# AvalonEnjoyer/pytorch-ViT-paper-replication

Hardware: AMD Instinct MI355X
Metric: images/sec (whole node) ViT-B/16 224px bf16 at 1/2/4/8 MI355X (higher is better)
Workload: dtype bf16; 1 GPU; model=ViT-B/16, global_batch=256, per_gpu_batch=256, seq_len=197, image_size=224, parallelism=dp1, impl=fused, grad_transport=none, optimizer=Adam(wd=0.03 decay group) + clip 1.0 + warmup/linear-decay LR, dropout=0.1 (mlp, embedding)

## Files before the change

### pytorch_vit_paper_replication_amd/csrc/layernorm.hip

```cpp
#include "common.h"
#include "kernels.h"

namespace pvr {
namespace {

template <int MAXCH>
__global__ void __launch_bounds__(256) ln_fwd_kernel(const uint16_t* __restrict__ x, int64_t x_stride,
                                                      const float* __restrict__ w, const float* __restrict__ b,
                                                      uint16_t* __restrict__ y, int64_t y_stride,
                                                      float* __restrict__ mean_out, float* __restrict__ rstd_out,
                                                      int rows, int D, float eps) {
  const int lane = threadIdx.x & 63;
  const int row = blockIdx.x * 4 + (threadIdx.x >> 6);
  if (row >= rows) return;
  const int nch = D >> 3;
  PVR_ASSERT((D & 7) == 0 && nch <= 64 * MAXCH);
  const uint16_t* xr = x + (int64_t)row * x_stride;
  float v[MAXCH][8];
  float s = 0.f;
#pragma unroll
  for (int i = 0; i < MAXCH; ++i) {
    const int c = lane + 64 * i;
    if (c < nch) {
      const uint4 q = *(const uint4*)(xr + c * 8);
      const uint32_t u[4] = {q.x, q.y, q.z, q.w};
#pragma unroll
      for (int j = 0; j < 4; ++j) {
        v[i][2 * j] = bf2f(u[j] & 0xFFFF);
        v[i][2 * j + 1] = bf2f(u[j] >> 16);
      }
#pragma unroll
      for (int j = 0; j < 8; ++j) s += v[i][j];
    } else {
#pragma unroll
      for (int j = 0; j < 8; ++j) v[i][j] = 0.f;
    }
  }
  const float mean = wave_sum(s) / D;
  float ss = 0.f;
#pragma unroll
  for (int i = 0; i < MAXCH; ++i) {
    const int c = lane + 64 * i;
    if (c < nch) {
#pragma unroll
      for (int j = 0; j < 8; ++j) {
        const float d = v[i][j] - mean;
        ss += d * d;
      }
    }
  }
  const float rstd = rsqrtf(wave_sum(ss) / D + eps);
  uint16_t* yr = y + (int64_t)row * y_stride;
#pragma unroll
  for (int i = 0; i < MAXCH; ++i) {
    const int c = lane + 64 * i;
    if (c < nch) {
      const float4 w0 = *(const float4*)(w + c * 8), w1 = *(const float4*)(w + c * 8 + 4);
      const float4 b0 = *(const float4*)(b + c * 8), b1 = *(const float4*)(b + c * 8 + 4);
      const float ww[8] = {w0.x, w0.y, w0.z, w0.w, w1.x, w1.y, w1.z, w1.w};
      const float bb[8] = {b0.x, b0.y, b0.z, b0.w, b1.x, b1.y, b1.z, b1.w};
      float o[8];
#pragma unroll
      for (int j = 0; j < 8; ++j) o[j] = (v[i][j] - mean) * rstd * ww[j] + bb[j];
      uint4 q;
      q.x = pack2bf(o[0], o[1]); q.y = pack2bf(o[2], o[3]);
      q.z = pack2bf(o[4], o[5]); q.w = pack2bf(o[6], o[7]);
      *(uint4*)(yr + c * 8) = q;
    }
  }
  if (lane == 0) {
    mean_out[row] = mean;
    rstd_out[row] = rstd;
  }
}

template <int MAXCH>
__global__ void __launch_bounds__(256) ln_fwd_q8_kernel(const uint16_t* __restrict__ x, int64_t x_stride,
                                                        const float* __restrict__ w, const float* __restrict__ b,
                                                        uint16_t* __restrict__ y, int64_t y_stride, uint8_t* __restrict__ yq,
                                                        int64_t q_stride, const float* __restrict__ qscale,
                                                        unsigned* __restrict__ amax, float* __restrict__ mean_out,
                                                        float* __restrict__ rstd_out, int rows, int D, float eps) {
  __shared__ float wm[4];
  const int lane = threadIdx.x & 63;
  const int nch = D >> 3;
  const float qs = *qscale;
  float am = 0.f;
  for (int row = blockIdx.x * 4 + (int)(threadIdx.x >> 6); row < rows; row += gridDim.x * 4) {
    const uint16_t* xr = x + (int64_t)row * x_stride;
    float v[MAXCH][8];
    float s = 0.f;
#pragma unroll
    for (int i = 0; i < MAXCH; ++i) {
      const int c = lane + 64 * i;
      if (c < nch) {
        const uint4 q = *(const uint4*)(xr + c * 8);
        const uint32_t u[4] = {q.x, q.y, q.z, q.w};
#pragma unroll
        for (int j = 0; j < 4; ++j) {
          v[i][2 * j] = bf2f(u[j] & 0xFFFF);
          v[i][2 * j + 1] = bf2f(u[j] >> 16);
        }
#pragma unroll
        for (int j = 0; j < 8; ++j) s += v[i][j];
      } else {
#pragma unroll
        for (int j = 0; j < 8; ++j) v[i][j] = 0.f;
      }
    }
    const float mean = wave_sum(s) / D;
    float ss = 0.f;
#pragma unroll
    for (int i = 0; i < MAXCH; ++i) {
      const int c = lane + 64 * i;
      if (c < nch) {
#pragma unroll
        for (int j = 0; j < 8; ++j) {
          const float d = v[i][j] - mean;
          ss += d * d;
        }
      }
    }
    const float rstd = rsqrtf(wave_sum(ss) / D + eps);
    uint16_t* yr = y ? y + (int64_t)row * y_stride : nullptr;
    uint8_t* qr = yq + (int64_t)row * q_stride;
#pragma unroll
    for (int i = 0; i < MAXCH; ++i) {
      const int c = lane + 64 * i;
      if (c < nch) {
        const float4 w0 = *(const float4*)(w + c * 8), w1 = *(const float4*)(w + c * 8 + 4);
        const float4 b0 = *(const float4*)(b + c * 8), b1 = *(const float4*)(b + c * 8 + 4);
        const float ww[8] = {w0.x, w0.y, w0.z, w0.w, w1.x, w1.y, w1.z, w1.w};
        const float bb[8] = {b0.x, b0.y, b0.z, b0.w, b1.x, b1.y, b1.z, b1.w};
        float o[8];
        float vm = 0.f;
#pragma unroll
        for (int j = 0; j < 8; ++j) {
          o[j] = (v[i][j] - mean) * rstd * ww[j] + bb[j];
          vm = nan_max(vm, fabsf(o[j]));
        }
        am = nan_max(am, vm);
        uint4 q;
        q.x = pack2bf(o[0], o[1]); q.y = pack2bf(o[2], o[3]);
        q.z = pack2bf(o[4], o[5]); q.w = pack2bf(o[6], o[7]);
        if (yr) *(uint4*)(yr + c * 8) = q;
        *(uint2*)(qr + c * 8) = pack8_fp8_fast<0>(o, qs, vm);
      }
    }
    if (lane == 0) {
      mean_out[row] = mean;
      rstd_out[row] = rstd;
    }
  }
  am = wave_max_nan(am);
  if (lane == 0) wm[threadIdx.x >> 6] = am;
  __syncthreads();
  if (threadIdx.x == 0) {
    const float m = nan_max(nan_max(wm[0], wm[1]), nan_max(wm[2], wm[3]));
    if (!(m <= 0.f)) atomicMax(amax, __float_as_uint(m));
  }
}

PVR_DEV void load8(const uint16_t* p, float* o) {
  const uint4 q = *(const uint4*)p;
  const uint32_t u[4] = {q.x, q.y, q.z, q.w};
#pragma unroll
  for (int j = 0; j < 4; ++j) {
    o[2 * j] = bf2f(u[j] & 0xFFFF);
    o[2 * j + 1] = bf2f(u[j] >> 16);
  }
}

template <int W>
struct RowVec;
template <>
struct RowVec<8> {
  uint32_t u[4];
  PVR_DEV void load(const uint16_t* p) { const uint4 q = *(const uint4*)p; u[0] = q.x; u[1] = q.y; u[2] = q.z; u[3] = q.w; }
  PVR_DEV void store(uint16_t* p) const { *(uint4*)p = make_uint4(u[0], u[1], u[2], u[3]); }
  PVR_DEV void zero() { u[0] = u[1] = u[2] = u[3] = 0u; }
};
template <>
struct RowVec<4> {
  uint32_t u[2];
  PVR_DEV void load(const uint16_t* p) { const uint2 q = *(const uint2*)p; u[0] = q.x; u[1] = q.y; }
  PVR_DEV void store(uint16_t* p) const { *(uint2*)p = make_uint2(u[0], u[1]); }
  PVR_DEV void zero() { u[0] = u[1] = 0u; }
};

template <int MAXCH, int W, bool Q8, bool SP, bool DP = false>
__global__ void __launch_bounds__(256) ln_bwd_kernel(const uint16_t* __restrict__ dy, int64_t dy_stride,
                                                      const uint16_t* __restrict__ x, int64_t x_stride,
                                                      const float* __restrict__ mean, const float* __restrict__ rstd,
                                                      const float* __restrict__ w,
                                                      const uint16_t* __restrict__ dres, int64_t dres_stride,
                                                      uint16_t* __restrict__ dx, int64_t dx_stride,
                                                      float* __restrict__ dw, float* __restrict__ db, float* __restrict__ dsum,
                                                      float* __restrict__ part,
                                                      uint16_t* __restrict__ dz, int64_t dz_stride,
                                                      const uint64_t* __restrict__ seed_ptr, uint64_t seed_off, uint32_t thr,
                                                      float dscale, int dz_nostore, uint8_t* __restrict__ qout, int64_t q_stride,
                                                      const float* __restrict__ qscale, unsigned* __restrict__ amax, int qfmt,
                                                      int rows, int D, int dres_every,
                                                      const uint64_t* __restrict__ dp_seed_ptr, uint64_t dp_off, uint32_t dp_thr,
                                                      float dp_scale, int dp_rows) {
  __shared__ float red[4][MAXCH * 64 * W > 1280 ? 1280 : MAXCH * 64 * W];
  __shared__ float qred[4];
  const float qs = Q8 ? *qscale : 1.f;
  float qam = 0.f;
  const int lane = threadIdx.x & 63, wave = threadIdx.x >> 6;
  const int nch = D / W;
  float gw[MAXCH][W], gb[MAXCH][W], gs[MAXCH][W];
#pragma unroll
  for (int i = 0; i < MAXCH; ++i)
#pragma unroll
    for (int j = 0; j < W; ++j) gw[i][j] = gb[i][j] = gs[i][j] = 0.f;

  const int stride = gridDim.x * 4;
  RowVec<W> cx[MAXCH], cdy[MAXCH], cr[MAXCH];
  auto load_row = [&](int row, RowVec<W> (&qx)[MAXCH], RowVec<W> (&qd)[MAXCH], RowVec<W> (&qr)[MAXCH]) {
    const int rr = min(row, rows - 1);
#pragma unroll
    for (int i = 0; i < MAXCH; ++i) {
      const int c = min(lane + 64 * i, nch - 1);
      qx[i].load(x + (int64_t)rr * x_stride + c * W);
      qd[i].load(dy + (int64_t)rr * dy_stride + c * W);
      if constexpr (SP) {
        qr[i].load(dres + (int64_t)(rr / dres_every) * dres_stride + c * W);
        if (rr % dres_every) qr[i].zero();
      } else if (dres)
        qr[i].load(dres + (int64_t)rr * dres_stride + c * W);
      else
        qr[i].zero();
    }
  };
  float wreg[MAXCH][W];
#pragma unroll
  for (int i = 0; i < MAXCH; ++i) {
    const int c = min(lane + 64 * i, nch - 1);
#pragma unroll
    for (int j = 0; j < W; j += 4) {
      const float4 w4 = *(const float4*)(w + c * W + j);
      wreg[i][j] = w4.x; wreg[i][j + 1] = w4.y; wreg[i][j + 2] = w4.z; wreg[i][j + 3] = w4.w;
    }
  }
  const uint64_t seed = dz && (!DP || thr) ? *seed_ptr + seed_off : 0ull;
  uint32_t dkey = 0u;
  float dfk = 0.f;
  if constexpr (DP) {
    dkey = rng_key(*dp_seed_ptr + dp_off);
    dfk = (thr ? dscale : 1.f) * dp_scale;
  }
  int row = blockIdx.x * 4 + wave;
  load_row(row, cx, cdy, cr);
  float cmu = row < rows ? mean[row] : 0.f, crs = row < rows ? rstd[row] : 0.f;
  for (; row < rows; row += stride) {
    RowVec<W> nx[MAXCH], ndy[MAXCH], nr[MAXCH];
    load_row(row + stride, nx, ndy, nr);
    const int rn = min(row + stride, rows - 1);
    const float nmu = mean[rn], nrs = rstd[rn];
    const float mu = cmu, rs = crs;
    auto xhat = [&](int i, int j) { return (bf2f(j & 1 ? cx[i].u[j >> 1] >> 16 : cx[i].u[j >> 1] & 0xFFFF) - mu) * rs; };
    auto dyv = [&](int i, int j) { return bf2f(j & 1 ? cdy[i].u[j >> 1] >> 16 : cdy[i].u[j >> 1] & 0xFFFF); };
    float s1 = 0.f, s2 = 0.f;
#pragma unroll
    for (int i = 0; i < MAXCH; ++i) {
      const int c = lane + 64 * i;
      if (c < nch) {
#pragma unroll
        for (int j = 0; j < W; ++j) {
          const float xh = xhat(i, j), dv = dyv(i, j);
          const float g = dv * wreg[i][j];
          s1 += g;
          s2 += g * xh;
          gw[i][j] += dv * xh;
          gb[i][j] += dv;
        }
      }
    }
    const float c1 = wave_sum(s1) / D, c2 = wave_sum(s2) / D;
#pragma unroll
    for (int i = 0; i < MAXCH; ++i) {
      const int c = lane + 64 * i;
      if (c < nch) {
        float o[W];
#pragma unroll
        for (int j = 0; j < W; ++j) o[j] = (dyv(i, j) * wreg[i][j] - c1 - xhat(i, j) * c2) * rs;
        if (dres) {
#pragma unroll
          for (int j = 0; j < W; ++j) o[j] += bf2f(j & 1 ? cr[i].u[j >> 1] >> 16 : cr[i].u[j >> 1] & 0xFFFF);
        }
        RowVec<W> q;
#pragma unroll
        for (int j = 0; j < W; j += 2) q.u[j >> 1] = pack2bf(o[j], o[j + 1]);
        q.store(dx + (int64_t)row * dx_stride + c * W);
        if (dz) {
          if constexpr (DP) {
            const float rf = rng_keep_32(dkey, (uint32_t)row / (uint32_t)dp_rows, dp_thr) ? dfk : 0.f;
#pragma unroll
            for (int j = 0; j < W; j += 2) {
              bool k0 = true, k1 = true;
              if (thr) rng_keep2(seed, (uint64_t)row * D + c * W + j, thr, k0, k1);
              o[j] = k0 ? o[j] * rf : 0.f;
              o[j + 1] = k1 ? o[j + 1] * rf : 0.f;
            }
          } else {
#pragma unroll
            for (int j = 0; j < W; j += 2) {
              bool k0, k1;
              rng_keep2(seed, (uint64_t)row * D + c * W + j, thr, k0, k1);
              o[j] = k0 ? o[j] * dscale : 0.f;
              o[j + 1] = k1 ? o[j + 1] * dscale : 0.f;
            }
          }
          if (!Q8 || !dz_nostore) {
#pragma unroll
            for (int j = 0; j < W; j += 2) q.u[j >> 1] = pack2bf(o[j], o[j + 1]);
            q.store(dz + (int64_t)row * dz_stride + c * W);
          }
          if constexpr (DP) {
#pragma unroll
            for (int j = 0; j < W; ++j) o[j] = bf2f(j & 1 ? q.u[j >> 1] >> 16 : q.u[j >> 1] & 0xFFFF);
          }
        }
        if constexpr (Q8) {
          uint32_t b4[W / 4];
          float vm = 0.f;
#pragma unroll
          for (int j = 0; j < W; ++j) vm = nan_max(vm, fabsf(o[j]));
          qam = nan_max(qam, vm);
          if (qfmt ? fp8_direct_ok<1>(vm, qs) : fp8_direct_ok<0>(vm, qs)) {
#pragma unroll
            for (int j = 0; j < W; j += 4)
              b4[j >> 2] = qfmt ? pack4_fp8_direct<1>(o[j] * qs, o[j + 1] * qs, o[j + 2] * qs, o[j + 3] * qs)
                                : pack4_fp8_direct<0>(o[j] * qs, o[j + 1] * qs, o[j + 2] * qs, o[j + 3] * qs);
          } else {
#pragma unroll
            for (int j = 0; j < W; j += 4) b4[j >> 2] = pack4_fp8_rt(qfmt, o[j] * qs, o[j + 1] * qs, o[j + 2] * qs, o[j + 3] * qs);
          }
          uint8_t* qp = qout + (int64_t)row * q_stride + c * W;
          if constexpr (W == 8)
            *(uint2*)qp = make_uint2(b4[0], b4[1]);
          else
            *(uint32_t*)qp = b4[0];
        }
#pragma unroll
        for (int j = 0; j < W; ++j) gs[i][j] += o[j];
      }
    }
#pragma unroll
    for (int i = 0; i < MAXCH; ++i) {
      cx[i] = nx[i];
      cdy[i] = ndy[i];
      cr[i] = nr[i];
    }
    cmu = nmu;
    crs = nrs;
  }
  float* outs[3] = {dw, db, dsum};
#pragma unroll
  for (int qn = 0; qn < 3; ++qn) {
    if (!outs[qn]) continue;
    if (qn) __syncthreads();
#pragma unroll
    for (int i = 0; i < MAXCH; ++i) {
      const int c = lane + 64 * i;
      if (c < nch) {
#pragma unroll
        for (int j = 0; j < W; ++j) red[wave][c * W + j] = qn == 0 ? gw[i][j] : (qn == 1 ? gb[i][j] : gs[i][j]);
      }
    }
    __syncthreads();
    if (part) {
      float* pr = part + ((int64_t)blockIdx.x * 3 + qn) * D;
      for (int col = threadIdx.x; col < D; col += 256) pr[col] = red[0][col] + red[1][col] + red[2][col] + red[3][col];
    } else {
      for (int col = threadIdx.x; col < D; col += 256)
        atomicAdd(outs[qn] + col, red[0][col] + red[1][col] + red[2][col] + red[3][col]);
    }
  }
  if constexpr (Q8) {
    qam = wave_max_nan(qam);
    if (lane == 0) qred[wave] = qam;
    __syncthreads();
    if (threadIdx.x == 0) {
      const float m = nan_max(nan_max(qred[0], qred[1]), nan_max(qred[2], qred[3]));
      if (!(m <= 0.f)) atomicMax(amax, __float_as_uint(m));
    }
  }
}

}
}

static int device_cus() {
  static const int n = [] {
    int dev = 0, cus = 0;
    if (hipGetDevice(&dev) != hipSuccess || hipDeviceGetAttribute(&cus, hipDeviceAttributeMultiprocessorCount, dev) != hipSuccess ||
        cus <= 0)
      cus = 256;
    return cus;
  }();
  return n;
}

extern "C" hipError_t pvr_layernorm_fwd(const uint16_t* x, int64_t x_stride, const float* w, const float* b,
                                        uint16_t* y, int64_t y_stride, float* mean, float* rstd, int rows, int D,
                                        float eps, hipStream_t s) {
  using namespace pvr;
  if (rows <= 0) return hipSuccess;
  if (D % 8 != 0 || D > 2048) return hipErrorInvalidValue;
  const dim3 grid((rows + 3) / 4), block(256);
  const int maxch = (D / 8 + 63) / 64;
  switch (maxch) {
    case 1: hipLaunchKernelGGL(ln_fwd_kernel<1>, grid, block, 0, s, x, x_stride, w, b, y, y_stride, mean, rstd, rows, D, eps); break;
    case 2: hipLaunchKernelGGL(ln_fwd_kernel<2>, grid, block, 0, s, x, x_stride, w, b, y, y_stride, mean, rstd, rows, D, eps); break;
    case 3: hipLaunchKernelGGL(ln_fwd_kernel<3>, grid, block, 0, s, x, x_stride, w, b, y, y_stride, mean, rstd, rows, D, eps); break;
    default: hipLaunchKernelGGL(ln_fwd_kernel<4>, grid, block, 0, s, x, x_stride, w, b, y, y_stride, mean, rstd, rows, D, eps); break;
  }
  return hipGetLastError();
}

static int g_ln_q8_blocks_per_cu = 4;
extern "C" void pvr_set_ln_fwd_q8_grid(int per_cu) { g_ln_q8_blocks_per_cu = per_cu < 1 ? 1 : per_cu > 64 ? 64 : per_cu; }

extern "C" hipError_t pvr_layernorm_fwd_q8(const uint16_t* x, int64_t x_stride, const float* w, const float* b, uint16_t* y,
                                           int64_t y_stride, pvr::Fp8Copy q, float* mean, float* rstd, int rows, int D, float eps,
                                           hipStream_t s) {
  using namespace pvr;
  if (rows <= 0) return hipSuccess;
  if (D % 8 != 0 || D > 2048 || q.ld % 8 != 0) return hipErrorInvalidValue;
  int nblk = (rows + 3) / 4;
  const int cap = g_ln_q8_blocks_per_cu * device_cus();
  if (nblk > cap) nblk = cap;
  const dim3 grid(nblk), block(256);
  switch ((D / 8 + 63) / 64) {
    case 1: hipLaunchKernelGGL(ln_fwd_q8_kernel<1>, grid, block, 0, s, x, x_stride, w, b, y, y_stride, q.out, q.ld, q.scale, q.amax, mean, rstd, rows, D, eps); break;
    case 2: hipLaunchKernelGGL(ln_fwd_q8_kernel<2>, grid, block, 0, s, x, x_stride, w, b, y, y_stride, q.out, q.ld, q.scale, q.amax, mean, rstd, rows, D, eps); break;
    case 3: hipLaunchKernelGGL(ln_fwd_q8_kernel<3>, grid, block, 0, s, x, x_stride, w, b, y, y_stride, q.out, q.ld, q.scale, q.amax, mean, rstd, rows, D, eps); break;
    default: hipLaunchKernelGGL(ln_fwd_q8_kernel<4>, grid, block, 0, s, x, x_stride, w, b, y, y_stride, q.out, q.ld, q.scale, q.amax, mean, rstd, rows, D, eps); break;
  }
  return hipGetLastError();
}

extern "C" int pvr_layernorm_bwd_blocks(int rows, int D) {
  const bool use_w4 = (D / 4) % 64 == 0 && (D / 8) % 64 != 0 && D / 4 <= 64 * 5;
  const int cap = use_w4 && D == 768 ? device_cus() * 3 : 1024;
  const int nblk = (rows + 3) / 4;
  return nblk > cap ? cap : nblk;
}

extern "C" hipError_t pvr_layernorm_bwd(const pvr::LnBwdParams* pp, hipStream_t s) {
  using namespace pvr;
  const LnBwdParams& p = *pp;
  const DropSite& d = p.drop;
  const Fp8Copy& q = p.q;
  const int rows = p.rows, D = p.D;
  if (rows <= 0) return hipSuccess;
  if (q.fmt != 0 && q.fmt != 1) return hipErrorInvalidValue;
  const DropSite& dp = p.dpath;
  const bool has_drop = d.seed && d.thr, has_dp = dp.seed && dp.thr;
  if (D % 8 != 0 || D > 1280 || (p.dz && !has_drop && !has_dp)) return hipErrorInvalidValue;
  if (has_dp && (!p.dz || q.out || p.dp_rows < 1 || dp.thr > 65535u)) return hipErrorInvalidValue;
  if (q.out && (!q.scale || !q.amax || q.ld % 8 != 0 || reinterpret_cast<uintptr_t>(q.out) % 8 != 0)) return hipErrorInvalidValue;
  if (p.dz_nostore && (!p.dz || !q.out)) return hipErrorInvalidValue;
  const bool sparse = p.dres && p.dres_every > 1;
  if (p.dres_every < 0 || (sparse && q.out)) return hipErrorInvalidValue;
  const bool use_w4 = (D / 4) % 64 == 0 && (D / 8) % 64 != 0 && D / 4 <= 64 * 5;
  const int nblk = pvr_layernorm_bwd_blocks(rows, D);
  float* part = p.dw || p.db || p.dsum ? p.part : nullptr;
  const dim3 grid(nblk), block(256);
#define PVR_LN_BWD(MC, W)                                                                                                   \
  hipLaunchKernelGGL(q.out ? (ln_bwd_kernel<MC, W, true, false>) : has_dp ? (sparse ? (ln_bwd_kernel<MC, W, false, true, true>) : (ln_bwd_kernel<MC, W, false, false, true>)) : sparse ? (ln_bwd_kernel<MC, W, false, true>) : (ln_bwd_kernel<MC, W, false, false>), grid, block, 0, s, p.dy, p.dy_stride, p.x, p.x_stride, p.mean, p.rstd, p.w, p.dres, p.dres_stride, p.dx, \
                     p.dx_stride, p.dw, p.db, p.dsum, part, p.dz, p.dz_stride, d.seed, d.offset, d.thr, d.scale, p.dz_nostore, q.out, q.ld, q.scale, q.amax, \
                     q.fmt, rows, D, p.dres_every, dp.seed, dp.offset, has_dp ? dp.thr : 0u, dp.scale, p.dp_rows)
  if (use_w4) {
    switch (D / 256) {
      case 3: PVR_LN_BWD(3, 4); break;
      case 5: PVR_LN_BWD(5, 4); break;
      default: PVR_LN_BWD(1, 4); break;
    }
  } else {
    const int maxch = (D / 8 + 63) / 64;
    switch (maxch) {
      case 1: PVR_LN_BWD(1, 8); break;
      case 2: PVR_LN_BWD(2, 8); break;
      default: PVR_LN_BWD(3, 8); break;
    }
  }
#undef PVR_LN_BWD
  const hipError_t e = hipGetLastError();
  if (e != hipSuccess || !part) return e;
  return pvr_rows_reduce(part, nblk, 3 * D, D, p.dw, p.db, p.dsum, s);
}
```

Baseline: 7877 images/sec.

## Add two-rows-per-wave LayerNorm forward/backward kernels for D=768

Adds specialized LayerNorm forward (plain and fp8) and backward kernels for D=768 in which each 64-lane wave processes two rows at once. With 96 8-element chunks per row, this gives every lane 3 chunks and no idle lanes. The kernels use a persistent grid capped at resident occupancy, prefetch the next row pair into registers, keep weights and bias in registers or LDS, and use packed v2f math. The backward kernel uses 8 waves per block for the dw/db partial reduction. The cost is more register pressure, larger LDS use, and extra code paths to keep correct for tail rows and the dropout/fp8 variants.

```diff
diff --git a/pytorch_vit_paper_replication_amd/csrc/layernorm.hip b/pytorch_vit_paper_replication_amd/csrc/layernorm.hip
--- a/pytorch_vit_paper_replication_amd/csrc/layernorm.hip
+++ b/pytorch_vit_paper_replication_amd/csrc/layernorm.hip
@@ -1,3 +1,5 @@
+#include <type_traits>
+
 #include "common.h"
 #include "kernels.h"
 
@@ -71,6 +73,144 @@
   if (lane == 0) {
     mean_out[row] = mean;
     rstd_out[row] = rstd;
+  }
+}
+
+PVR_DEV v2f bf2x(uint32_t u) { return (v2f){__uint_as_float(u << 16), __uint_as_float(u & 0xFFFF0000u)}; }
+PVR_DEV v2f splat(float a) { return (v2f){a, a}; }
+
+template <int NP>
+struct PairMap {
+  static constexpr int NCH = 32 * NP;
+  int ck[NP];
+  bool r1[NP];
+  PVR_DEV explicit PairMap(int lane) {
+#pragma unroll
+    for (int k = 0; k < NP; ++k) {
+      const int c = lane + 64 * k;
+      r1[k] = c >= NCH;
+      ck[k] = r1[k] ? c - NCH : c;
+    }
+  }
+  template <class T>
+  PVR_DEV T pick(int k, T a, T b) const { return r1[k] ? b : a; }
+};
+
+template <int NP, bool Q8>
+__global__ void __launch_bounds__(256) ln_fwd_pair_kernel(const uint16_t* __restrict__ x, int64_t x_stride,
+                                                           const float* __restrict__ w, const float* __restrict__ b,
+                                                           uint16_t* __restrict__ y, int64_t y_stride,
+                                                           uint8_t* __restrict__ yq, int64_t q_stride,
+                                                           const float* __restrict__ qscale, unsigned* __restrict__ amax,
+                                                           float* __restrict__ mean_out, float* __restrict__ rstd_out,
+                                                           int rows, float eps) {
+  constexpr int D = 256 * NP;
+  __shared__ float wm[4];
+  const float qs = Q8 ? *qscale : 1.f;
+  float am = 0.f;
+  const int lane = threadIdx.x & 63, wave = __builtin_amdgcn_readfirstlane(threadIdx.x >> 6);
+  const PairMap<NP> pm(lane);
+  v2f wv[NP][4], bv[NP][4];
+#pragma unroll
+  for (int k = 0; k < NP; ++k) {
+#pragma unroll
+    for (int j = 0; j < 4; j += 2) {
+      const float4 w4 = *(const float4*)(w + pm.ck[k] * 8 + 2 * j), b4 = *(const float4*)(b + pm.ck[k] * 8 + 2 * j);
+      wv[k][j] = (v2f){w4.x, w4.y}; wv[k][j + 1] = (v2f){w4.z, w4.w};
+      bv[k][j] = (v2f){b4.x, b4.y}; bv[k][j + 1] = (v2f){b4.z, b4.w};
+    }
+  }
+  const int npairs = (rows + 1) >> 1, stride = gridDim.x * 4;
+  auto load_pair = [&](int pair, uint4 (&q)[NP]) {
+    const int ra = 2 * min(pair, npairs - 1), rb = min(ra + 1, rows - 1);
+    const uint16_t *xa = x + (int64_t)ra * x_stride, *xb = x + (int64_t)rb * x_stride;
+#pragma unroll
+    for (int k = 0; k < NP; ++k) q[k] = *(const uint4*)(pm.pick(k, xa, xb) + pm.ck[k] * 8);
+  };
+  int pair = blockIdx.x * 4 + wave;
+  uint4 cur[NP];
+  load_pair(pair, cur);
+  auto body = [&](auto tail) {
+    constexpr bool has_b = !decltype(tail)::value;
+    uint4 nxt[NP];
+    load_pair(pair + stride, nxt);
+    v2f v[NP][4];
+    float sa = 0.f, sb = 0.f;
+#pragma unroll
+    for (int k = 0; k < NP; ++k) {
+      const uint32_t u[4] = {cur[k].x, cur[k].y, cur[k].z, cur[k].w};
+      v2f t = {0.f, 0.f};
+#pragma unroll
+      for (int j = 0; j < 4; ++j) {
+        v[k][j] = bf2x(u[j]);
+        t += v[k][j];
+      }
+      const float s = t.x + t.y;
+      sa += pm.pick(k, s, 0.f);
+      sb += pm.pick(k, 0.f, s);
+    }
+    const float ma = wave_sum(sa) / D, mb = wave_sum(sb) / D;
+    float qa = 0.f, qb = 0.f;
+#pragma unroll
+    for (int k = 0; k < NP; ++k) {
+      const v2f m = splat(pm.pick(k, ma, mb));
+      v2f t = {0.f, 0.f};
+#pragma unroll
+      for (int j = 0; j < 4; ++j) {
+        const v2f d = v[k][j] - m;
+        t = __builtin_elementwise_fma(d, d, t);
+      }
+      const float s = t.x + t.y;
+      qa += pm.pick(k, s, 0.f);
+      qb += pm.pick(k, 0.f, s);
+    }
+    const float ra_ = rsqrtf(wave_sum(qa) / D + eps), rb_ = rsqrtf(wave_sum(qb) / D + eps);
+    const int row0 = 2 * pair;
+#pragma unroll
+    for (int k = 0; k < NP; ++k) {
+      const v2f m = splat(pm.pick(k, ma, mb)), r = splat(pm.pick(k, ra_, rb_));
+      uint32_t o[4];
+      float e8[8];
+#pragma unroll
+      for (int j = 0; j < 4; ++j) {
+        const v2f e = __builtin_elementwise_fma((v[k][j] - m) * r, wv[k][j], bv[k][j]);
+        o[j] = pack2bf(e.x, e.y);
+        e8[2 * j] = e.x;
+        e8[2 * j + 1] = e.y;
+      }
+      const bool live = !pm.r1[k] || has_b;
+      const int64_t row = row0 + (pm.r1[k] ? 1 : 0);
+      if (live && (!Q8 || y)) *(uint4*)(y + row * y_stride + pm.ck[k] * 8) = make_uint4(o[0], o[1], o[2], o[3]);
+      if constexpr (Q8) {
+        float vm = 0.f;
+#pragma unroll
+        for (int j = 0; j < 8; ++j) vm = nan_max(vm, fabsf(e8[j]));
+        am = nan_max(am, vm);
+        if (live) *(uint2*)(yq + row * q_stride + pm.ck[k] * 8) = pack8_fp8_fast<0>(e8, qs, vm);
+      }
+    }
+    if (lane == 0) {
+      mean_out[row0] = ma;
+      rstd_out[row0] = ra_;
+      if (has_b) {
+        mean_out[row0 + 1] = mb;
+        rstd_out[row0 + 1] = rb_;
+      }
+    }
+#pragma unroll
+    for (int k = 0; k < NP; ++k) cur[k] = nxt[k];
+  };
+  const int nfull = rows >> 1;
+  for (; pair < nfull; pair += stride) body(std::false_type{});
+  if (pair < npairs) body(std::true_type{});
+  if constexpr (Q8) {
+    am = wave_max_nan(am);
+    if (lane == 0) wm[wave] = am;
+    __syncthreads();
+    if (threadIdx.x == 0) {
+      const float m = nan_max(nan_max(wm[0], wm[1]), nan_max(wm[2], wm[3]));
+      if (!(m <= 0.f)) atomicMax(amax, __float_as_uint(m));
+    }
   }
 }
 
@@ -390,6 +530,252 @@
   }
 }
 
+template <int NP, int NW, bool Q8, bool SP, bool DP>
+__global__ void __launch_bounds__(64 * NW) ln_bwd_pair_kernel(const uint16_t* __restrict__ dy, int64_t dy_stride,
+                                                           const uint16_t* __restrict__ x, int64_t x_stride,
+                                                           const float* __restrict__ mean, const float* __restrict__ rstd,
+                                                           const float* __restrict__ w,
+                                                           const uint16_t* __restrict__ dres, int64_t dres_stride,
+                                                           uint16_t* __restrict__ dx, int64_t dx_stride,
+                                                           float* __restrict__ dw, float* __restrict__ db, float* __restrict__ dsum,
+                                                           float* __restrict__ part,
+                                                           uint16_t* __restrict__ dz, int64_t dz_stride,
+                                                           const uint64_t* __restrict__ seed_ptr, uint64_t seed_off, uint32_t thr,
+                                                           float dscale, int dz_nostore, uint8_t* __restrict__ qout,
+                                                           int64_t q_stride, const float* __restrict__ qscale,
+                                                           unsigned* __restrict__ amax, int qfmt, int rows, int dres_every,
+                                                           const uint64_t* __restrict__ dp_seed_ptr, uint64_t dp_off, uint32_t dp_thr,
+                                                           float dp_scale, int dp_rows) {
+  constexpr int D = 256 * NP;
+  __shared__ float red[2 * NW][D];
+  __shared__ float wl[D];
+  __shared__ float qred[NW];
+  const float qs = Q8 ? *qscale : 1.f;
+  float qam = 0.f;
+  const int lane = threadIdx.x & 63, wave = __builtin_amdgcn_readfirstlane(threadIdx.x >> 6);
+  const PairMap<NP> pm(lane);
+  for (int i = threadIdx.x * 4; i < D; i += 256 * NW) *(float4*)(wl + i) = *(const float4*)(w + i);
+  __syncthreads();
+  v2f gw[NP][4], gb[NP][4], gs[NP][4];
+#pragma unroll
+  for (int k = 0; k < NP; ++k)
+#pragma unroll
+    for (int j = 0; j < 4; ++j) gw[k][j] = gb[k][j] = gs[k][j] = splat(0.f);
+
+  const int npairs = (rows + 1) >> 1, stride = gridDim.x * NW;
+  RowVec<8> cx[NP], cdy[NP], cr[NP];
+  auto load_pair = [&](int pair, RowVec<8> (&qx)[NP], RowVec<8> (&qd)[NP], RowVec<8> (&qr)[NP]) {
+    const int ra = 2 * min(pair, npairs - 1), rb = min(ra + 1, rows - 1);
+    const uint16_t *xa = x + (int64_t)ra * x_stride, *xb = x + (int64_t)rb * x_stride;
+    const uint16_t *da = dy + (int64_t)ra * dy_stride, *dB = dy + (int64_t)rb * dy_stride;
+    const uint16_t *ea = nullptr, *eb = nullptr;
+    if (dres) {
+      ea = dres + (int64_t)(SP ? ra / dres_every : ra) * dres_stride;
+      eb = dres + (int64_t)(SP ? rb / dres_every : rb) * dres_stride;
+    }
+#pragma unroll
+    for (int k = 0; k < NP; ++k) {
+      qx[k].load(pm.pick(k, xa, xb) + pm.ck[k] * 8);
+      qd[k].load(pm.pick(k, da, dB) + pm.ck[k] * 8);
+      if (dres)
+        qr[k].load(pm.pick(k, ea, eb) + pm.ck[k] * 8);
+      else
+        qr[k].zero();
+    }
+  };
+  const uint64_t seed = dz && (!DP || thr) ? *seed_ptr + seed_off : 0ull;
+  uint32_t dkey = 0u;
+  float dfk = 0.f;
+  if constexpr (DP) {
+    dkey = rng_key(*dp_seed_ptr + dp_off);
+    dfk = (thr ? dscale : 1.f) * dp_scale;
+  }
+  int pair = blockIdx.x * NW + wave;
+  load_pair(pair, cx, cdy, cr);
+  float cmua = 0.f, cmub = 0.f, crsa = 0.f, crsb = 0.f;
+  if (pair < npairs) {
+    const int ra = 2 * pair, rb = min(ra + 1, rows - 1);
+    cmua = mean[ra]; cmub = mean[rb];
+    crsa = rstd[ra]; crsb = rstd[rb];
+  }
+  auto body = [&](auto tail) {
+    constexpr bool has_b = !decltype(tail)::value;
+    RowVec<8> nx[NP], ndy[NP], nr[NP];
+    load_pair(pair + stride, nx, ndy, nr);
+    const int rna = 2 * min(pair + stride, npairs - 1), rnb = min(rna + 1, rows - 1);
+    const float nmua = mean[rna], nmub = mean[rnb], nrsa = rstd[rna], nrsb = rstd[rnb];
+    const int row0 = 2 * pair;
+    if (!has_b) {
+#pragma unroll
+      for (int k = 0; k < NP; ++k)
+#pragma unroll
+        for (int j = 0; j < 4; ++j) {
+          cdy[k].u[j] = pm.r1[k] ? 0u : cdy[k].u[j];
+          cr[k].u[j] = pm.r1[k] ? 0u : cr[k].u[j];
+        }
+    }
+    float s1a = 0.f, s1b = 0.f, s2a = 0.f, s2b = 0.f;
+#pragma unroll
+    for (int k = 0; k < NP; ++k) {
+      const v2f mu = splat(pm.pick(k, cmua, cmub)), rs = splat(pm.pick(k, crsa, crsb));
+      v2f t1 = splat(0.f), t2 = splat(0.f);
+#pragma unroll
+      for (int j = 0; j < 4; ++j) {
+        const v2f wv = *(const v2f*)(wl + pm.ck[k] * 8 + 2 * j);
+        const v2f xh = (bf2x(cx[k].u[j]) - mu) * rs, dv = bf2x(cdy[k].u[j]);
+        const v2f g = dv * wv;
+        t1 = __builtin_elementwise_fma(dv, wv, t1);
+        t2 = __builtin_elementwise_fma(g, xh, t2);
+        gw[k][j] = __builtin_elementwise_fma(dv, xh, gw[k][j]);
+        gb[k][j] += dv;
+      }
+#pragma unroll
+      for (int j = 0; j < 4; ++j) asm volatile("" : "+v"(gw[k][j]), "+v"(gb[k][j]));
+      const float u1 = t1.x + t1.y, u2 = t2.x + t2.y;
+      s1a += pm.pick(k, u1, 0.f); s1b += pm.pick(k, 0.f, u1);
+      s2a += pm.pick(k, u2, 0.f); s2b += pm.pick(k, 0.f, u2);
+    }
+    const float c1a = wave_sum(s1a) / D, c1b = wave_sum(s1b) / D, c2a = wave_sum(s2a) / D, c2b = wave_sum(s2b) / D;
+#pragma unroll
+    for (int k = 0; k < NP; ++k)
+#pragma unroll
+      for (int j = 0; j < 4; ++j) asm volatile("" : "+v"(cx[k].u[j]), "+v"(cdy[k].u[j]));
+    bool resa = true, resb = true;
+    if constexpr (SP) {
+      resa = row0 % dres_every == 0;
+      resb = (row0 + 1) % dres_every == 0;
+    }
+    float rfa = 0.f, rfb = 0.f;
+    if constexpr (DP) {
+      if (dz) {
+        rfa = rng_keep_32(dkey, (uint32_t)row0 / (uint32_t)dp_rows, dp_thr) ? dfk : 0.f;
+        rfb = rng_keep_32(dkey, (uint32_t)(row0 + 1) / (uint32_t)dp_rows, dp_thr) ? dfk : 0.f;
+      }
+    }
+#pragma unroll
+    for (int k = 0; k < NP; ++k) {
+      const v2f mu = splat(pm.pick(k, cmua, cmub)), rs = splat(pm.pick(k, crsa, crsb));
+      const v2f c1 = splat(pm.pick(k, c1a, c1b)), c2 = splat(pm.pick(k, c2a, c2b));
+      const int row = row0 + (pm.r1[k] ? 1 : 0);
+      const bool live = !pm.r1[k] || has_b;
+      v2f o[4];
+#pragma unroll
+      for (int j = 0; j < 4; ++j) {
+        const v2f wv = *(const v2f*)(wl + pm.ck[k] * 8 + 2 * j);
+        const v2f xh = (bf2x(cx[k].u[j]) - mu) * rs, dv = bf2x(cdy[k].u[j]);
+        o[j] = __builtin_elementwise_fma(-xh, c2, __builtin_elementwise_fma(dv, wv, -c1)) * rs;
+      }
+      if (dres) {
+        const bool res = pm.pick(k, resa, resb);
+#pragma unroll
+        for (int j = 0; j < 4; ++j) {
+          const v2f r = bf2x(cr[k].u[j]);
+          o[j] += SP ? (res ? r : splat(0.f)) : r;
+        }
+      }
+      RowVec<8> q;
+#pragma unroll
+      for (int j = 0; j < 4; ++j) q.u[j] = pack2bf(o[j].x, o[j].y);
+      if (live) q.store(dx + (int64_t)row * dx_stride + pm.ck[k] * 8);
+      if (dz) {
+        const uint64_t idx = (uint64_t)row * D + pm.ck[k] * 8;
+        if constexpr (DP) {
+          const v2f rf = splat(pm.pick(k, rfa, rfb));
+#pragma unroll
+          for (int j = 0; j < 4; ++j) {
+            bool k0 = true, k1 = true;
+            if (thr) rng_keep2(seed, idx + 2 * j, thr, k0, k1);
+            o[j] *= rf;
+            o[j] = (v2f){k0 ? o[j].x : 0.f, k1 ? o[j].y : 0.f};
+          }
+        } else {
+          const v2f ds = splat(dscale);
+#pragma unroll
+          for (int j = 0; j < 4; ++j) {
+            bool k0, k1;
+            rng_keep2(seed, idx + 2 * j, thr, k0, k1);
+            o[j] *= ds;
+            o[j] = (v2f){k0 ? o[j].x : 0.f, k1 ? o[j].y : 0.f};
+          }
+        }
+        if (!Q8 || !dz_nostore) {
+#pragma unroll
+          for (int j = 0; j < 4; ++j) q.u[j] = pack2bf(o[j].x, o[j].y);
+          if (live) q.store(dz + (int64_t)row * dz_stride + pm.ck[k] * 8);
+        }
+        if constexpr (DP) {
+#pragma unroll
+          for (int j = 0; j < 4; ++j) o[j] = bf2x(q.u[j]);
+        }
+      }
+      if constexpr (Q8) {
+        float vm = 0.f;
+#pragma unroll
+        for (int j = 0; j < 4; ++j) vm = nan_max(vm, nan_max(fabsf(o[j].x), fabsf(o[j].y)));
+        qam = nan_max(qam, vm);
+        uint32_t b4[2];
+        if (qfmt ? fp8_direct_ok<1>(vm, qs) : fp8_direct_ok<0>(vm, qs)) {
+#pragma unroll
+          for (int j = 0; j < 4; j += 2)
+            b4[j >> 1] = qfmt ? pack4_fp8_direct<1>(o[j].x * qs, o[j].y * qs, o[j + 1].x * qs, o[j + 1].y * qs)
+                              : pack4_fp8_direct<0>(o[j].x * qs, o[j].y * qs, o[j + 1].x * qs, o[j + 1].y * qs);
+        } else {
+#pragma unroll
+          for (int j = 0; j < 4; j += 2) b4[j >> 1] = pack4_fp8_rt(qfmt, o[j].x * qs, o[j].y * qs, o[j + 1].x * qs, o[j + 1].y * qs);
+        }
+        if (live) *(uint2*)(qout + (int64_t)row * q_stride + pm.ck[k] * 8) = make_uint2(b4[0], b4[1]);
+      }
+#pragma unroll
+      for (int j = 0; j < 4; ++j) gs[k][j] += o[j];
+    }
+#pragma unroll
+    for (int k = 0; k < NP; ++k) {
+      cx[k] = nx[k];
+      cdy[k] = ndy[k];
+      cr[k] = nr[k];
+    }
+    cmua = nmua; cmub = nmub;
+    crsa = nrsa; crsb = nrsb;
+  };
+  const int nfull = rows >> 1;
+  for (; pair < nfull; pair += stride) body(std::false_type{});
+  if (pair < npairs) body(std::true_type{});
+  float* outs[3] = {dw, db, dsum};
+#pragma unroll
+  for (int qn = 0; qn < 3; ++qn) {
+    if (!outs[qn]) continue;
+    if (qn) __syncthreads();
+#pragma unroll
+    for (int k = 0; k < NP; ++k) {
+      float* rr = red[wave * 2 + (pm.r1[k] ? 1 : 0)] + pm.ck[k] * 8;
+#pragma unroll
+      for (int j = 0; j < 4; ++j) *(v2f*)(rr + 2 * j) = qn == 0 ? gw[k][j] : (qn == 1 ? gb[k][j] : gs[k][j]);
+    }
+    __syncthreads();
+    float* pr = part ? part + ((int64_t)blockIdx.x * 3 + qn) * D : nullptr;
+    for (int col = threadIdx.x; col < D; col += 64 * NW) {
+      float t = red[0][col];
+#pragma unroll
+      for (int r = 1; r < 2 * NW; ++r) t += red[r][col];
+      if (part)
+        pr[col] = t;
+      else
+        atomicAdd(outs[qn] + col, t);
+    }
+  }
+  if constexpr (Q8) {
+    qam = wave_max_nan(qam);
+    if (lane == 0) qred[wave] = qam;
+    __syncthreads();
+    if (threadIdx.x == 0) {
+      float m = qred[0];
+#pragma unroll
+      for (int r = 1; r < NW; ++r) m = nan_max(m, qred[r]);
+      if (!(m <= 0.f)) atomicMax(amax, __float_as_uint(m));
+    }
+  }
+}
+
 }
 }
 
@@ -404,12 +790,26 @@
   return n;
 }
 
+template <class K>
+static int resident_blocks(K kernel, int threads) {
+  int per_cu = 0;
+  if (hipOccupancyMaxActiveBlocksPerMultiprocessor(&per_cu, kernel, threads, 0) != hipSuccess || per_cu < 1) per_cu = 1;
+  return per_cu * device_cus();
+}
+
 extern "C" hipError_t pvr_layernorm_fwd(const uint16_t* x, int64_t x_stride, const float* w, const float* b,
                                         uint16_t* y, int64_t y_stride, float* mean, float* rstd, int rows, int D,
                                         float eps, hipStream_t s) {
   using namespace pvr;
   if (rows <= 0) return hipSuccess;
   if (D % 8 != 0 || D > 2048) return hipErrorInvalidValue;
+  if (D == 768) {
+    static const int cap = resident_blocks(ln_fwd_pair_kernel<3, false>, 256);
+    const int nblk = ((rows + 1) / 2 + 3) / 4;
+    hipLaunchKernelGGL((ln_fwd_pair_kernel<3, false>), dim3(nblk > cap ? cap : nblk), dim3(256), 0, s, x, x_stride, w, b, y, y_stride,
+                       nullptr, 0, nullptr, nullptr, mean, rstd, rows, eps);
+    return hipGetLastError();
+  }
   const dim3 grid((rows + 3) / 4), block(256);
   const int maxch = (D / 8 + 63) / 64;
   switch (maxch) {
@@ -430,8 +830,16 @@
   using namespace pvr;
   if (rows <= 0) return hipSuccess;
   if (D % 8 != 0 || D > 2048 || q.ld % 8 != 0) return hipErrorInvalidValue;
+  const int cap = g_ln_q8_blocks_per_cu * device_cus();
+  if (D == 768) {
+    static const int res = resident_blocks(ln_fwd_pair_kernel<3, true>, 256);
+    int nb = ((rows + 1) / 2 + 3) / 4;
+    nb = nb > cap ? cap : nb;
+    hipLaunchKernelGGL((ln_fwd_pair_kernel<3, true>), dim3(nb > res ? res : nb), dim3(256), 0, s, x, x_stride, w, b, y, y_stride,
+                       q.out, q.ld, q.scale, q.amax, mean, rstd, rows, eps);
+    return hipGetLastError();
+  }
   int nblk = (rows + 3) / 4;
-  const int cap = g_ln_q8_blocks_per_cu * device_cus();
   if (nblk > cap) nblk = cap;
   const dim3 grid(nblk), block(256);
   switch ((D / 8 + 63) / 64) {
@@ -443,11 +851,16 @@
   return hipGetLastError();
 }
 
+static constexpr int kLnPairWaves = 8;
+
 extern "C" int pvr_layernorm_bwd_blocks(int rows, int D) {
-  const bool use_w4 = (D / 4) % 64 == 0 && (D / 8) % 64 != 0 && D / 4 <= 64 * 5;
-  const int cap = use_w4 && D == 768 ? device_cus() * 3 : 1024;
+  if (D == 768) {
+    static const int cap = resident_blocks(pvr::ln_bwd_pair_kernel<3, kLnPairWaves, false, false, false>, 64 * kLnPairWaves);
+    const int nblk = ((rows + 1) / 2 + kLnPairWaves - 1) / kLnPairWaves;
+    return nblk > cap ? cap : nblk;
+  }
   const int nblk = (rows + 3) / 4;
-  return nblk > cap ? cap : nblk;
+  return nblk > 1024 ? 1024 : nblk;
 }
 
 extern "C" hipError_t pvr_layernorm_bwd(const pvr::LnBwdParams* pp, hipStream_t s) {
@@ -474,9 +887,21 @@
   hipLaunchKernelGGL(q.out ? (ln_bwd_kernel<MC, W, true, false>) : has_dp ? (sparse ? (ln_bwd_kernel<MC, W, false, true, true>) : (ln_bwd_kernel<MC, W, false, false, true>)) : sparse ? (ln_bwd_kernel<MC, W, false, true>) : (ln_bwd_kernel<MC, W, false, false>), grid, block, 0, s, p.dy, p.dy_stride, p.x, p.x_stride, p.mean, p.rstd, p.w, p.dres, p.dres_stride, p.dx, \
                      p.dx_stride, p.dw, p.db, p.dsum, part, p.dz, p.dz_stride, d.seed, d.offset, d.thr, d.scale, p.dz_nostore, q.out, q.ld, q.scale, q.amax, \
                      q.fmt, rows, D, p.dres_every, dp.seed, dp.offset, has_dp ? dp.thr : 0u, dp.scale, p.dp_rows)
-  if (use_w4) {
+#define PVR_LN_BWD_PAIR(Q8, SP, DP)                                                                                          \
+  hipLaunchKernelGGL((ln_bwd_pair_kernel<3, kLnPairWaves, Q8, SP, DP>), grid, dim3(64 * kLnPairWaves), 0, s, p.dy, p.dy_stride, p.x, p.x_stride, p.mean, p.rstd, p.w, \
+                     p.dres, p.dres_stride, p.dx, p.dx_stride, p.dw, p.db, p.dsum, part, p.dz, p.dz_stride, d.seed, d.offset,    \
+                     d.thr, d.scale, p.dz_nostore, q.out, q.ld, q.scale, q.amax, q.fmt, rows, p.dres_every, dp.seed, dp.offset,   \
+                     has_dp ? dp.thr : 0u, dp.scale, p.dp_rows)
+  if (D == 768) {
+    if (q.out) {
+      PVR_LN_BWD_PAIR(true, false, false);
+    } else if (has_dp) {
+      if (sparse) PVR_LN_BWD_PAIR(false, true, true); else PVR_LN_BWD_PAIR(false, false, true);
+    } else {
+      if (sparse) PVR_LN_BWD_PAIR(false, true, false); else PVR_LN_BWD_PAIR(false, false, false);
+    }
+  } else if (use_w4) {
     switch (D / 256) {
-      case 3: PVR_LN_BWD(3, 4); break;
       case 5: PVR_LN_BWD(5, 4); break;
       default: PVR_LN_BWD(1, 4); break;
     }
@@ -489,6 +914,7 @@
     }
   }
 #undef PVR_LN_BWD
+#undef PVR_LN_BWD_PAIR
   const hipError_t e = hipGetLastError();
   if (e != hipSuccess || !part) return e;
   return pvr_rows_reduce(part, nblk, 3 * D, D, p.dw, p.db, p.dsum, s);
```

Result: no change. 7908 images/sec, median of 6 (+0.4%).
